# duanzhiihao/myDetection

Measured on AMD Instinct MI355X. Metric: images/sec at batch 32, 640x640, YOLOv3-80 (backbone -> FPN -> head -> decode -> NMS), higher is better.
Workload: dtype f32; 1 GPU; yolov3_80 (Darknet-53 + YOLOv3 FPN/head + decode + conf 0.005/top-512/NMS 0.45), batch 32/GPU, 640x640, random-init calibrated weights, hipGraph replay (1 batch lane per GPU); global_batch=32, image_size=640, parallelism=dp1, batch_lanes=1, batch_lanes_rule=model.batch_lanes_hint, passes=153, exchange=none

## Files before the change

include/mydet.h:

```cpp
#ifndef MYDET_H
#define MYDET_H

#include <stdint.h>

#ifdef __cplusplus
extern "C" {
#endif

#define MYDET_ABI_VERSION 2

#define MYDET_E_BADARG   (-1)
#define MYDET_E_UNSUPP   (-2)

#define MYDET_ACT_NONE   0
#define MYDET_ACT_LEAKY  1
#define MYDET_ACT_SWISH  2

int mydet_abi_version(void);

int mydet_conv2d_igemm_f32(const float *x, int64_t ldx, const float *w,
                           const float *scale, const float *shift,
                           const float *residual, int64_t ldr, const float *a_gate,
                           void *workspace, int64_t workspace_bytes,
                           float *y, int64_t ldy,
                           int B, int H, int W, int Cin, int Cout,
                           int KH, int KW, int stride, int pad_t, int pad_l,
                           int Ho, int Wo, int act, void *stream);

int64_t mydet_wino_weights_floats(int Cout, int Cin);
int mydet_wino_weights_f32(const float *w_ohwi, int Cout, int Cin, float *u, void *stream);
int mydet_conv2d_wino_f32(const float *x, int64_t ldx, const float *u, const float *scale, const float *shift,
                          const float *residual, int64_t ldr, void *workspace, int64_t workspace_bytes, float *y,
                          int64_t ldy, int B, int H, int W, int Cin, int Cout, int act, void *stream);

int mydet_conv2d_stem_f32(const float *x, int64_t sxb, int64_t sxc, int64_t sxh, int64_t sxw,
                          const float *w ,
                          const float *scale, const float *shift,
                          float *y, int64_t ldy,
                          int B, int H, int W, int Cout, int stride, int pad_t, int pad_l,
                          int Ho, int Wo, int act, void *stream);

#define MYDET_SE_EPOCH_WORDS 1024
typedef struct {
    const float *w1, *b1, *w2t, *b2;
    float *gate, *hpart;
    int Cse;
    int64_t hpart_bytes;
} mydet_se_tail;
int mydet_dwconv_slices(int Ho, int Wo, int C, int K, int stride);
int mydet_dwconv_se_groups(int Ho, int Wo, int C, int K, int stride);
int mydet_dwconv_f32(const float *x, int64_t ldx, const float *w, const float *scale, const float *shift,
                     float *y, int64_t ldy, int B, int H, int W, int C, int K, int stride, int pad_t, int pad_l,
                     int Ho, int Wo, int act, float *se_partial, int S, const mydet_se_tail *se, void *stream);

int mydet_channel_sums_f32(const float *x, int64_t ldx, int B, int H, int W, int C, float *partial, int S,
                           void *stream);

int mydet_se_gate_f32(float *partial, int S, int B, int HW, int C, const float *w1, const float *b1, int Cse,
                      const float *w2t, const float *b2, float *gate, void *stream);

int mydet_maxpool3s2_f32(const float *x, int64_t ldx, float *y, int64_t ldy, int B, int H, int W, int C,
                         int Ho, int Wo, void *stream);

int mydet_bifpn_fuse_f32(int n, const float *in0, int64_t ld0, int mode0, const float *in1, int64_t ld1, int mode1,
                         const float *in2, int64_t ld2, int mode2, const float *weights, float *y, int64_t ldy,
                         int B, int H, int W, int C, void *stream);

int mydet_upsample_concat_f32(const float *a, int64_t lda, int Ha, int Wa, int C1,
                              const float *b, int64_t ldb, int C2,
                              float *y, int64_t ldy, int B, int Ho, int Wo, void *stream);

int mydet_conv1x1_upcat_f32(const float *x_lo, int64_t ld_lo, int C_lo, const float *x_hi, int64_t ld_hi, int C_hi,
                            const float *w, const float *scale, const float *shift, void *workspace,
                            int64_t workspace_bytes, float *y, int64_t ldy, int B, int H, int W, int Cout, int act,
                            void *stream);

int64_t mydet_split_bf16_elems(int Cout, int K);
int mydet_split_bf16_f32(const float *w, int Cout, int K, uint16_t *planes, void *stream);
int mydet_conv2d_igemm_b3_f32(const float *x, int64_t ldx, const uint16_t *w_planes, const float *scale, const float *shift,
                              const float *residual, int64_t ldr, const float *a_gate, void *workspace, int64_t workspace_bytes, float *y,
                              int64_t ldy, int B, int H, int W, int Cin, int Cout, int KH, int KW, int stride, int pad_t,
                              int pad_l, int Ho, int Wo, int act, void *stream);
int mydet_conv3x3_p3_f32(const float *x, int64_t ldx, const uint16_t *w_planes, const float *scale, const float *shift,
                         const float *residual, int64_t ldr, float *y, int64_t ldy, int B, int H, int W, int Cin, int Cout,
                         int stride, int act, void *stream);
int mydet_conv_b3_reload_tuning(void);

int mydet_conv_igemm_occupancy(int cfg, int *assumed);

int mydet_space_to_depth_f32(const float *x, int64_t sb, int64_t sc, int64_t sh, int64_t sw, float *y, int64_t ldy,
                             int B, int C, int H, int W, void *stream);

int mydet_spp_concat_f32(const float *x, int64_t ldx, float *y, int64_t ldy, int B, int H, int W, int C, int k0, int k1,
                         int k2, void *stream);

#define MYDET_DECODE_YOLO   0
#define MYDET_DECODE_RETINA 1
#define MYDET_DECODE_FCOS   2
#define MYDET_DECODE_RAPID  3
typedef struct mydet_decode_level {
    const float *box; int64_t ldbox;
    const float *cls; int64_t ldcls;
    const float *anchors_wh;
    int H, W;
    float stride;
    int64_t n_off;
} mydet_decode_level;
int mydet_decode_levels_f32(int mode, int nlevels, const mydet_decode_level *levels, int box_astride, int box_c0,
                            int cls_astride, int cls_c0, int conf_c0, int A, int C, int B, int img_h, int img_w,
                            float *bbox, int64_t *class_idx, float *score, int64_t N, void *stream);
int mydet_decode_uv5_levels_f32(int nlevels, const mydet_decode_level *levels, int box_astride, int box_c0,
                                int cls_astride, int cls_c0, int conf_c0, int A, int C, int B, int img_h, int img_w,
                                float *bbox, int64_t *class_idx, float *score, int64_t N, void *stream);
int mydet_decode_f32(int mode,
                     const float *box, int64_t ldbox, int box_astride, int box_c0,
                     const float *cls, int64_t ldcls, int cls_astride, int cls_c0, int conf_c0,
                     const float *anchors_wh, int A, int C,
                     int B, int H, int W, float stride, int img_h, int img_w,
                     float *bbox, int64_t *class_idx, float *score, int64_t N, int64_t n_off,
                     void *stream);

int mydet_postprocess_f32(const float *bbox, const int64_t *class_idx, const float *score,
                          int B, int64_t N, float conf_thres, double nms_thres, int topk,
                          int32_t *count, float *out_bbox, int64_t *out_class, float *out_score,
                          int32_t *out_index, void *scratch, void *stream);

#define MYDET_COUNT_BAD_CLASS (-1)
#define MYDET_REC_TOPK   512
#define MYDET_REC_COUNT  0
#define MYDET_REC_BBOX   4
#define MYDET_REC_SCORE  (MYDET_REC_BBOX + 4 * MYDET_REC_TOPK)
#define MYDET_REC_CLASS  (MYDET_REC_SCORE + MYDET_REC_TOPK)
#define MYDET_REC_INDEX  (MYDET_REC_CLASS + 2 * MYDET_REC_TOPK)
#define MYDET_REC_WORDS  (MYDET_REC_INDEX + MYDET_REC_TOPK)
int mydet_postprocess_records_f32(const float *bbox, const int64_t *class_idx, const float *score,
                                  int B, int64_t N, float conf_thres, double nms_thres,
                                  int32_t *records, void *scratch, void *stream);

#define MYDET_REC_ANGLE     MYDET_REC_WORDS
#define MYDET_REC_ROT_WORDS (MYDET_REC_WORDS + MYDET_REC_TOPK)
int mydet_postprocess_rot_f32(const float *bbox, const int64_t *class_idx, const float *score,
                              int B, int64_t N, float conf_thres, double nms_thres, int topk,
                              int32_t *count, float *out_bbox, int64_t *out_class, float *out_score,
                              int32_t *out_index, void *scratch, void *stream);
int mydet_postprocess_records_rot_f32(const float *bbox, const int64_t *class_idx, const float *score,
                                      int B, int64_t N, float conf_thres, double nms_thres,
                                      int32_t *records, void *scratch, void *stream);

int64_t mydet_wino4_weights_floats(int Cout, int Cin);
int mydet_wino4_weights_f32(const float *w, int Cout, int Cin, float *u, void *stream);
int64_t mydet_wino4_workspace_bytes(int B, int H, int W, int Cin, int Cout);
int mydet_wino4_reload_tuning(void);
int mydet_conv2d_wino4_f32(const float *x, int64_t ldx, const float *u, const float *scale, const float *shift,
                           const float *residual, int64_t ldr, float *ws, int64_t ws_bytes, float *y, int64_t ldy,
                           int B, int H, int W, int Cin, int Cout, int act, void *stream);
int mydet_wino4_tail_plan(int B, int H, int W, int Cin, int Cout, int slots, int32_t *out);

int mydet_resize_bilinear_u8(const unsigned char *src, int H, int W, int64_t src_row_bytes, unsigned char *dst, int oh,
                             int ow, int64_t dst_row_bytes, const int32_t *bounds_x, const int32_t *kx, int ksx,
                             const int32_t *bounds_y, const int32_t *ky, int ksy, void *stream);

int mydet_bboxes_to_original_batched_f32(float *bbox, int64_t bbox_stride, const int32_t *count, int64_t count_stride,
                                         int B, int K, const float *pad_info, void *stream);
int mydet_detections_to_json_f64(const float *bbox, int64_t bbox_stride, const float *score, int64_t score_stride,
                                 const int64_t *cls, int64_t cls_stride, const int32_t *count, int64_t count_stride,
                                 int B, int K, const int64_t *cat_table, int n_cat, double *out, int64_t *out_cat,
                                 void *stream);

// ... 68 lines not shown
```

mydetection_amd/_lib.py:

```python
import ctypes
import os

_HERE = os.path.dirname(os.path.abspath(__file__))
LIB_PATH = os.environ.get('MYDET_LIB_PATH') or os.path.join(_HERE, 'lib', 'libmydet_hip.so')

c_int, c_i64, c_f32, c_f64, c_ptr = ctypes.c_int, ctypes.c_int64, ctypes.c_float, ctypes.c_double, ctypes.c_void_p

SIGNATURES = {
    'mydet_abi_version': [],
    'mydet_conv2d_igemm_f32': [c_ptr, c_i64, c_ptr, c_ptr, c_ptr, c_ptr, c_i64, c_ptr, c_ptr, c_i64, c_ptr, c_i64]
    + [c_int] * 13 + [c_ptr],
    'mydet_wino_weights_floats': [c_int, c_int],
    'mydet_wino_weights_f32': [c_ptr, c_int, c_int, c_ptr, c_ptr],
    'mydet_conv2d_wino_f32': [c_ptr, c_i64, c_ptr, c_ptr, c_ptr, c_ptr, c_i64, c_ptr, c_i64, c_ptr, c_i64] + [c_int] * 6
    + [c_ptr],
    'mydet_wino4_weights_floats': [c_int, c_int],
    'mydet_wino4_weights_f32': [c_ptr, c_int, c_int, c_ptr, c_ptr],
    'mydet_wino4_workspace_bytes': [c_int, c_int, c_int, c_int, c_int],
    'mydet_wino4_reload_tuning': [],
    'mydet_conv_b3_reload_tuning': [],
    'mydet_conv_igemm_occupancy': [c_int, c_ptr],
    'mydet_split_bf16_elems': [c_int, c_int],
    'mydet_split_bf16_f32': [c_ptr, c_int, c_int, c_ptr, c_ptr],
    'mydet_conv2d_igemm_b3_f32': [c_ptr, c_i64, c_ptr, c_ptr, c_ptr, c_ptr, c_i64, c_ptr, c_ptr, c_i64, c_ptr, c_i64] + [c_int] * 13 + [c_ptr],
    'mydet_conv3x3_p3_f32': [c_ptr, c_i64, c_ptr, c_ptr, c_ptr, c_ptr, c_i64, c_ptr, c_i64] + [c_int] * 7 + [c_ptr],
    'mydet_wino4_tail_plan': [c_int, c_int, c_int, c_int, c_int, c_int, c_ptr],
    'mydet_conv2d_wino4_f32': [c_ptr, c_i64, c_ptr, c_ptr, c_ptr, c_ptr, c_i64, c_ptr, c_i64, c_ptr, c_i64] + [c_int] * 6 + [c_ptr],
    'mydet_dwconv_slices': [c_int, c_int, c_int, c_int, c_int],
    'mydet_dwconv_se_groups': [c_int, c_int, c_int, c_int, c_int],
    'mydet_dwconv_f32': [c_ptr, c_i64, c_ptr, c_ptr, c_ptr, c_ptr, c_i64] + [c_int] * 11 + [c_ptr, c_int, c_ptr, c_ptr],
    'mydet_channel_sums_f32': [c_ptr, c_i64, c_int, c_int, c_int, c_int, c_ptr, c_int, c_ptr],
    'mydet_se_gate_f32': [c_ptr, c_int, c_int, c_int, c_int, c_ptr, c_ptr, c_int, c_ptr, c_ptr, c_ptr, c_ptr],
    'mydet_maxpool3s2_f32': [c_ptr, c_i64, c_ptr, c_i64] + [c_int] * 6 + [c_ptr],
    'mydet_bifpn_fuse_f32': [c_int, c_ptr, c_i64, c_int, c_ptr, c_i64, c_int, c_ptr, c_i64, c_int, c_ptr, c_ptr, c_i64,
                             c_int, c_int, c_int, c_int, c_ptr],
    'mydet_conv2d_stem_f32': [c_ptr, c_i64, c_i64, c_i64, c_i64, c_ptr, c_ptr, c_ptr, c_ptr, c_i64] + [c_int] * 10 + [c_ptr],
    'mydet_upsample_concat_f32': [c_ptr, c_i64, c_int, c_int, c_int, c_ptr, c_i64, c_int, c_ptr, c_i64, c_int, c_int,
                                  c_int, c_ptr],
    'mydet_conv1x1_upcat_f32': [c_ptr, c_i64, c_int, c_ptr, c_i64, c_int, c_ptr, c_ptr, c_ptr, c_ptr, c_i64, c_ptr, c_i64]
    + [c_int] * 5 + [c_ptr],
    'mydet_space_to_depth_f32': [c_ptr, c_i64, c_i64, c_i64, c_i64, c_ptr, c_i64, c_int, c_int, c_int, c_int, c_ptr],
    'mydet_spp_concat_f32': [c_ptr, c_i64, c_ptr, c_i64] + [c_int] * 7 + [c_ptr],
    'mydet_decode_levels_f32': [c_int, c_int, c_ptr, c_int, c_int, c_int, c_int, c_int, c_int, c_int, c_int, c_int, c_int,
                                c_ptr, c_ptr, c_ptr, c_i64, c_ptr],
    'mydet_decode_uv5_levels_f32': [c_int, c_ptr, c_int, c_int, c_int, c_int, c_int, c_int, c_int, c_int, c_int, c_int,
                                    c_ptr, c_ptr, c_ptr, c_i64, c_ptr],
    'mydet_decode_f32': [c_int, c_ptr, c_i64, c_int, c_int, c_ptr, c_i64, c_int, c_int, c_int, c_ptr, c_int, c_int,
                         c_int, c_int, c_int, c_f32, c_int, c_int, c_ptr, c_ptr, c_ptr, c_i64, c_i64, c_ptr],
    'mydet_postprocess_f32': [c_ptr, c_ptr, c_ptr, c_int, c_i64, c_f32, c_f64, c_int, c_ptr, c_ptr, c_ptr, c_ptr,
                              c_ptr, c_ptr, c_ptr],
    'mydet_postprocess_records_f32': [c_ptr, c_ptr, c_ptr, c_int, c_i64, c_f32, c_f64, c_ptr, c_ptr, c_ptr],
    'mydet_postprocess_rot_f32': [c_ptr, c_ptr, c_ptr, c_int, c_i64, c_f32, c_f64, c_int, c_ptr, c_ptr, c_ptr, c_ptr,
                                  c_ptr, c_ptr, c_ptr],
    'mydet_postprocess_records_rot_f32': [c_ptr, c_ptr, c_ptr, c_int, c_i64, c_f32, c_f64, c_ptr, c_ptr, c_ptr],
    'mydet_mbconv_tiles': [c_int, c_int, c_int],
    'mydet_mbconv_expand_dw_f32': [c_ptr, c_i64, c_ptr, c_ptr, c_ptr, c_ptr, c_ptr, c_i64] + [c_int] * 11 + [c_ptr, c_int, c_ptr, c_ptr],
    'mydet_sepconv_nodes_f32': [c_int, c_ptr, c_int, c_int, c_ptr],
    'mydet_stem_dw_f32': [c_ptr, c_i64, c_i64, c_i64, c_i64, c_ptr, c_ptr, c_ptr, c_ptr, c_ptr, c_i64, c_int, c_int, c_int, c_int,
                          c_int, c_int, c_int, c_int, c_ptr, c_int, c_ptr, c_ptr],
    'mydet_lr_tb_levels_f32': [c_int, c_ptr, c_int, c_int, c_ptr],
    'mydet_sepconv_decode_retina_f32': [c_int, c_ptr, c_int, c_int, c_int, c_int, c_int, c_int, c_ptr, c_ptr, c_ptr, c_i64, c_ptr],
    'mydet_bboxes_iou_f32': [c_ptr, c_int, c_ptr, c_int, c_int, c_ptr, c_ptr],
    'mydet_bboxes_to_original_batched_f32': [c_ptr, c_i64, c_ptr, c_i64, c_int, c_int, c_ptr, c_ptr],
    'mydet_detections_to_json_f64': [c_ptr, c_i64, c_ptr, c_i64, c_ptr, c_i64, c_ptr, c_i64, c_int, c_int, c_ptr, c_int, c_ptr, c_ptr, c_ptr],
    'mydet_resize_bilinear_u8': [c_ptr, c_int, c_int, c_i64, c_ptr, c_int, c_int, c_i64, c_ptr, c_ptr, c_int, c_ptr, c_ptr, c_int, c_ptr],
    'mydet_preprocess_u8_f32': [c_ptr, c_int, c_int, c_int, c_ptr, c_int, c_int, c_int, c_ptr, c_ptr, c_ptr],
    'mydet_cxcywh_to_x1y1x2y2_f32': [c_ptr, c_ptr, c_i64, c_int, c_ptr],
    'mydet_bboxes_to_original_f32': [c_ptr, c_i64, c_f32, c_f32, c_f32, c_f32, c_f32, c_f32, c_ptr],
}



RETURNS_I64 = {'mydet_wino_weights_floats', 'mydet_wino4_weights_floats', 'mydet_wino4_workspace_bytes', 'mydet_split_bf16_elems'}

REC_TOPK = 512
REC_COUNT, REC_BBOX = 0, 4
REC_SCORE = REC_BBOX + 4 * REC_TOPK
REC_CLASS = REC_SCORE + REC_TOPK
REC_INDEX = REC_CLASS + 2 * REC_TOPK
REC_WORDS = REC_INDEX + REC_TOPK
REC_ANGLE = REC_WORDS
REC_ROT_WORDS = REC_WORDS + REC_TOPK


class DecodeLevel(ctypes.Structure):
    _fields_ = [('box', c_ptr), ('ldbox', c_i64), ('cls', c_ptr), ('ldcls', c_i64), ('anchors_wh', c_ptr),
                ('H', c_int), ('W', c_int), ('stride', c_f32), ('n_off', c_i64)]


class SeTail(ctypes.Structure):
    _fields_ = [('w1', c_ptr), ('b1', c_ptr), ('w2t', c_ptr), ('b2', c_ptr), ('gate', c_ptr), ('hpart', c_ptr), ('Cse', c_int),
                ('hpart_bytes', c_i64)]


SE_EPOCH_WORDS = 1024
ABI_VERSION = 2


class SepconvNode(ctypes.Structure):
    _fields_ = [('inp', c_ptr * 3), ('ld', c_i64 * 3), ('mode', c_int * 3), ('n_in', c_int), ('fuse_weights', c_ptr),
                ('w_dw', c_ptr), ('w_pw_packed', c_ptr), ('scale', c_ptr), ('shift', c_ptr), ('y', c_ptr), ('ldy', c_i64),
                ('H', c_int), ('W', c_int), ('Cout', c_int), ('act', c_int)]


class SepconvDecodeNode(ctypes.Structure):
    _fields_ = [('node', SepconvNode), ('kind', c_int), ('stride', c_f32), ('anchors_wh', c_ptr), ('n_off', c_i64)]


# ... 47 lines not shown
```

mydetection_amd/models/backbones.py:

```python
import torch.nn as nn

from .. import ops
from .modules import ConvBn, ConvBnLeaky, DarkBlock


class Darknet53(nn.Module):
    def __init__(self, global_cfg):
        super().__init__()
        self.netlist = nn.ModuleList()
        in_ch = global_cfg.get('model.backbone.input_channels', 3)
        self.netlist.append(ConvBnLeaky(in_ch, 32, k=3, s=1))
        width = 32
        for n_blocks in (1, 2, 8, 8, 4):
            self.netlist.append(ConvBnLeaky(width, width * 2, k=3, s=2))
            width *= 2
            for _ in range(n_blocks):
                self.netlist.append(DarkBlock(in_out=width, hidden=width // 2))
        assert len(self.netlist) == 29

    def forward(self, x):
        feats = []
        for i, layer in enumerate(self.netlist):
            x = layer(x)
            if i in (14, 23, 28):
                feats.append(x)
        return feats


class UltralyticsBackbone(nn.Module):
    def __init__(self, global_cfg):
        super().__init__()
        import math
        from ..external.ultralytics.common import Focus, Bottleneck, BottleneckCSP, Conv, SPP
        depm = global_cfg['model.ultralytics.depth_muliple']
        chm = global_cfg['model.ultralytics.channel_muliple']
        ch = [int(math.ceil(c * chm / 8) * 8) for c in (64, 128, 256, 512, 1024)]

        def reps(n):
            return max(round(n * depm), 1)
        self.feature_chs = ch[2:]
        self.feature_strides = [8, 16, 32]
        self.netlist = nn.ModuleList()
        if global_cfg['model.ultralytics.first'] == 'Focus':
            assert global_cfg.get('general.input.frame_concatenation', 1) == 1
            self.netlist.append(Focus(3, ch[0], k=3))
        else:
            raise NotImplementedError()
        self.netlist.append(Conv(ch[0], ch[1], k=3, s=2))
        self.netlist.append(nn.Sequential(*[Bottleneck(ch[1], ch[1]) for _ in range(reps(3))]))
        self.netlist.append(Conv(ch[1], ch[2], k=3, s=2))
        self.netlist.append(BottleneckCSP(ch[2], ch[2], n=reps(9)))
        self.netlist.append(Conv(ch[2], ch[3], k=3, s=2))
        self.netlist.append(BottleneckCSP(ch[3], ch[3], n=reps(9)))
        self.netlist.append(Conv(ch[3], ch[4], k=3, s=2))
        self.netlist.append(SPP(ch[4], ch[4], k=[5, 9, 13]))
        self.netlist.append(BottleneckCSP(ch[4], ch[4], n=reps(6)))

    def forward(self, x):
        assert x.dim() == 4 and x.shape[2] % 32 == 0 and x.shape[3] % 32 == 0
        features = []
        for module in self.netlist:
            y = module(x)
            if y.shape[2:4] != x.shape[2:4]:
                assert y.shape[2] == x.shape[2] // 2
                features.append(x)
            x = y
        features.append(x)
        assert len(features) == 6
        return features[3:]


class _PoolAfter(ConvBn):
    def __init__(self, in_ch, out_ch, k, padding):
        super().__init__(in_ch, out_ch, k, padding)
        self.add_module('2', nn.MaxPool2d(3, stride=2, padding=1))

    def forward(self, x):
        return ops.maxpool3s2(ConvBn.forward(self, x))


class _MaxPool(nn.Module):
    def forward(self, x):
        return ops.maxpool3s2(x)


class EfNetBackbone(nn.Module):
    valid_names = {'efficientnet-b0', 'efficientnet-b1', 'efficientnet-b2', 'efficientnet-b3', 'efficientnet-b4',
                   'efficientnet-b5', 'efficientnet-b6'}

    def __init__(self, cfg: dict):
        super().__init__()
        model_name = cfg['model.backbone.name']
        assert model_name in self.valid_names, 'Unknown efficientnet model name'
        from ..external.efficientnet.model import EfficientNet
        efn = EfficientNet.from_name(model_name)
        self.model = efn
        efnet_chs = [efn._blocks_args[i].output_filters for i in [2, 4, 6]]
        if cfg['model.backbone.num_levels'] == 3:
            self.feature_chs = efnet_chs
            self.feature_strides = (8, 16, 32)
            self.C6C7 = False
        elif cfg['model.backbone.num_levels'] == 5:
            out_ch = cfg['model.backbone.C6C7_out_channels']
            downsample_layer = cfg.get('model.efficientnet.C6C7_downsample', 'maxpool')
            if downsample_layer == 'maxpool':
# ... 35 lines not shown
```

mydetection_amd/models/modules.py:

```python
import torch
import torch.nn as nn

from .. import ops


def _versions(*tensors):
    return tuple((t.data_ptr(), t._version) for t in tensors)


def prepare_conv(owner, slot, conv, bn, depthwise=False):
    tensors = [conv.weight] + ([bn.weight, bn.bias, bn.running_mean, bn.running_var] if bn is not None else [])
    if conv.bias is not None:
        tensors.append(conv.bias)
    key = _versions(*tensors)
    cache = owner.__dict__.setdefault('_prep_cache', {})
    hit = cache.get(slot)
    if hit is None or hit[0] != key:
        with torch.no_grad():
            w = conv.weight.detach().float()
            if depthwise:
                w = w.permute(2, 3, 0, 1).reshape(w.shape[2], w.shape[3], w.shape[0]).contiguous()
            else:
                w = w.permute(0, 2, 3, 1).contiguous()
            if bn is not None:
                inv = (bn.running_var.float() + bn.eps).sqrt().reciprocal()
                scale = (bn.weight.float() * inv).contiguous()
                shift = (bn.bias.float() - bn.running_mean.float() * scale).contiguous()
                if conv.bias is not None:
                    shift = (shift + conv.bias.float() * scale).contiguous()
            else:
                scale = None
                shift = conv.bias.detach().float().contiguous() if conv.bias is not None else None
        hit = (key, (w, scale, shift))
        cache[slot] = hit
    return hit[1]


def prepare_wino(owner, slot, w_ohwi):
    cache = owner.__dict__.setdefault('_prep_cache', {})
    hit = cache.get(slot)
    if hit is None or hit[0] is not w_ohwi:
        u = ops.wino_weights(w_ohwi) if ops.WINOGRAD else None
        u4 = ops.wino4_weights(w_ohwi) if ops.WINOGRAD and ops.WINOGRAD4 and w_ohwi.shape[3] >= ops.WINO4_MIN_CIN else None
        hit = (w_ohwi, (u, u4))
        cache[slot] = hit
    return hit[1]


def prepare_b3(owner, slot, w_ohwi):
    if not ops.SPLIT_BF16 or (w_ohwi.shape[3] % 16 and not (w_ohwi.shape[1] == 1 and w_ohwi.shape[2] == 1 and w_ohwi.shape[3] % 4 == 0)):
        return None
    cache = owner.__dict__.setdefault('_prep_cache', {})
    hit = cache.get(slot)
    if hit is None or hit[0] is not w_ohwi:
        hit = (w_ohwi, ops.split_bf16(w_ohwi))
        cache[slot] = hit
    return hit[1]


class FusedConvMixin:

    def _prepared(self, conv, bn):
        return prepare_conv(self, 'main', conv, bn)


class ConvBnLeaky(nn.Module, FusedConvMixin):
    def __init__(self, c1, c2, k=1, s=1):
        super().__init__()
        self.k, self.s = k, s
        self.conv = nn.Conv2d(c1, c2, k, s, padding=(k - 1) // 2, bias=False)
        self.bn = nn.BatchNorm2d(c2, eps=1e-5, momentum=0.01)

    def forward(self, x, residual=None, upcat_lo=None):
        if self.training:
            raise NotImplementedError('mydetection_amd implements the inference path only; call model.eval()')
        w, scale, shift = self._prepared(self.conv, self.bn)
        p = (self.k - 1) // 2
        if upcat_lo is not None:
            assert residual is None
            if self.k == 1 and self.s == 1:
                y = ops.conv1x1_upcat(upcat_lo, x, w, scale, shift, ops.ACT_LEAKY)
                if y is not None:
                    return y
            x = ops.upsample_concat(upcat_lo, tuple(x.shape[2:4]), x)
        if w.shape[3] == 3 and self.k == 3 and w.shape[0] == 32 and residual is None:
            return ops.conv2d_stem(x, w, scale, shift, self.s, (p, p, p, p), ops.ACT_LEAKY)
        u, u4 = prepare_wino(self, 'wino', w) if self.k == 3 and self.s == 1 else (None, None)
        b3 = prepare_b3(self, 'b3', w) if (u is None and u4 is None) or (self.k == 3 and w.shape[3] <= ops.P3_S1_MAX_CIN) else None
        return ops.conv2d(x, w, scale, shift, self.k, self.s, (p, p, p, p), ops.ACT_LEAKY, residual=residual, wino=u, wino4=u4, b3=b3)


class DarkBlock(nn.Module):
    def __init__(self, in_out, hidden):
        super().__init__()
        self.cbl_0 = ConvBnLeaky(in_out, hidden, k=1, s=1)
        self.cbl_1 = ConvBnLeaky(hidden, in_out, k=3, s=1)

    def forward(self, x):
        return self.cbl_1(self.cbl_0(x), residual=x)


class Swish(nn.Module):
    def forward(self, x):
        raise NotImplementedError('Swish is fused into the producing conv kernel on the inference path')


class SeparableConv2d(nn.Module):
    def __init__(self, in_ch, out_ch, kernel_size, stride, padding):
        super().__init__()
        self.k, self.s, self.p = kernel_size, stride, padding
        self.depthwise = nn.Conv2d(in_ch, in_ch, kernel_size, stride, padding=padding, groups=in_ch, bias=False)
        self.pointwise = nn.Conv2d(in_ch, out_ch, 1, 1, padding=0)

    def fusable(self):
        return (ops.FUSED_NODES and self.k == 3 and self.s == 1 and self.p == 1
                and self.depthwise.in_channels in ops.SEPCONV_CHANNELS and self.pointwise.out_channels % 4 == 0)

    def node(self, inputs, modes=None, fuse_weights=None, bn=None, act=ops.ACT_NONE, out=None):
        if self.training:
            raise NotImplementedError('mydetection_amd implements the inference path only; call model.eval()')
        wd, _, _ = prepare_conv(self, 'dw', self.depthwise, None, depthwise=True)
        wp, scale, shift = prepare_conv(self, ('pw', id(bn)), self.pointwise, bn)
        cache = self.__dict__.setdefault('_prep_cache', {})
        hit = cache.get(('pwk', id(bn)))
        if hit is None or hit[0] is not wp:
            hit = (wp, ops.pack_pointwise(wp))
            cache[('pwk', id(bn))] = hit
        return dict(inputs=list(inputs), modes=modes, fuse_weights=fuse_weights, w_dw=wd, w_pw=hit[1], scale=scale,
                    shift=shift, cout=self.pointwise.out_channels, act=act, out=out)

    def node_per_anchor(self, inputs, A, n_cls):
        nd = self.node(inputs)
        wp, _, shift = prepare_conv(self, ('pw', id(None)), self.pointwise, None)
        cache = self.__dict__.setdefault('_prep_cache', {})
        hit = cache.get(('pwk_anchor', A, n_cls))
        if hit is None or hit[0] is not wp:
            hit = (wp, ops.pack_pointwise_per_anchor(wp, shift, A, n_cls))
            cache[('pwk_anchor', A, n_cls)] = hit
        nd['w_pw'], nd['shift'] = hit[1]
        return nd

    def forward(self, x, bn=None, act=ops.ACT_NONE):
        if self.training:
            raise NotImplementedError('mydetection_amd implements the inference path only; call model.eval()')
        if self.fusable():
            return ops.sepconv_nodes([self.node([x], bn=bn, act=act)])[0]
        wd, _, _ = prepare_conv(self, 'dw', self.depthwise, None, depthwise=True)
        x = ops.dwconv(x, wd, None, None, self.k, self.s, (self.p,) * 4, ops.ACT_NONE)
        wp, scale, shift = prepare_conv(self, ('pw', id(bn)), self.pointwise, bn)
        return ops.conv2d(x, wp, scale, shift, 1, 1, (0, 0, 0, 0), act)


class ConvBn(nn.Sequential):
    def __init__(self, in_ch, out_ch, k=1, padding=0, eps=0.001):
        super().__init__(nn.Conv2d(in_ch, out_ch, k, stride=1, padding=padding),
                         nn.BatchNorm2d(out_ch, eps=eps, momentum=0.01))
        self.k, self.p = k, padding

    def forward(self, x):
        w, scale, shift = prepare_conv(self, 'main', self[0], self[1])
        u, u4 = prepare_wino(self, 'wino', w) if self.k == 3 and self.p == 1 else (None, None)
        return ops.conv2d(x, w, scale, shift, self.k, 1, (self.p,) * 4, ops.ACT_NONE, wino=u, wino4=u4)


class SpconvBn(nn.Sequential):
    def __init__(self, ch, swish):
        mods = [SeparableConv2d(ch, ch, 3, 1, padding=1), nn.BatchNorm2d(ch, eps=0.001, momentum=0.01)]
        if swish:
            mods.append(Swish())
        super().__init__(*mods)
        self.act = ops.ACT_SWISH if swish else ops.ACT_NONE

    def fusable(self):
        return self[0].fusable()
# ... 7 lines not shown
```

mydetection_amd/ops.py:

```python
import ctypes
import os
import threading

import numpy as np
import torch

from . import _lib

ACT_NONE, ACT_LEAKY, ACT_SWISH = 0, 1, 2
DECODE_YOLO, DECODE_RETINA, DECODE_FCOS, DECODE_RAPID = 0, 1, 2, 3
TOPK = 512


def _stream():
    return ctypes.c_void_p(torch.cuda.current_stream().cuda_stream)


class KernelTimer:

    def __init__(self, chain=False):
        self.spans = {}
        self.bytes = {}
        self.fused = {}
        self.chain = chain
# ... 305 lines not shown
            TIMER.stop(name, t0, 2.0 * B * Ho * Wo * Cout * 9 * Cin,
                       4.0 * (B * H * W * Cin + B * Ho * Wo * Cout * (2 if residual is not None else 1) + 9 * Cin * Cout))
        _lib.check(code, 'mydet_conv2d_wino_f32')
        return out
    ws = conv_workspace(x.device)
    if (b3 is not None and b3_takes(B * Ho * Wo, Cin, Cout, k, b3_min_rows, min_cout=B3_GATED_MIN_COUT if gate is not None else 128)
            and (gate is None or (k == 1 and act == ACT_NONE))):
        t0 = TIMER.start() if TIMER else None
        code = _lib.lib().mydet_conv2d_igemm_b3_f32(
            _ptr(x), ldx, _ptr(b3), _ptr(scale), _ptr(shift), _ptr(residual), ldr, _ptr(gate), _ptr(ws), ws.numel() * 4, _ptr(out), ldy,
            B, H, W, Cin, Cout, k, k, stride, pad[0], pad[1], Ho, Wo, act, _stream())
        if code != -2:
            if t0:
                name = f'conv_igemm_b3 {Cin}->{Cout} k{k}s{stride} {H}x{W}' if TIMER_DETAIL else 'conv_igemm_b3'
                b_in, b_out = 4.0 * B * H * W * Cin, 4.0 * B * Ho * Wo * Cout
                b_rest = 4.0 * (k * k * Cin * Cout) + (b_out if residual is not None else 0.0)
                TIMER.stop(name, t0, 2.0 * B * Ho * Wo * Cout * k * k * Cin, b_in + b_out + b_rest)
            _lib.check(code, 'mydet_conv2d_igemm_b3_f32')
            return out
    t0 = TIMER.start() if TIMER else None
    code = _lib.lib().mydet_conv2d_igemm_f32(
        _ptr(x), ldx, _ptr(w_ohwi), _ptr(scale), _ptr(shift), _ptr(residual), ldr, _ptr(gate),
        _ptr(ws), ws.numel() * 4 if ws is not None else 0, _ptr(out), ldy,
        B, H, W, Cin, Cout, k, k, stride, pad[0], pad[1], Ho, Wo, act, _stream())
    if t0:
        name = f'conv_igemm {Cin}->{Cout} k{k}s{stride} {H}x{W}' if TIMER_DETAIL else 'conv_igemm'
        b_in, b_out = 4.0 * B * H * W * Cin, 4.0 * B * Ho * Wo * Cout
        b_rest = 4.0 * (k * k * Cin * Cout) + (b_out if residual is not None else 0.0)
        TIMER.stop(name, t0, 2.0 * B * Ho * Wo * Cout * k * k * Cin, b_in + b_out + b_rest,
                   (0.0 if interior == 'in' else b_in) + (0.0 if interior == 'out' else b_out) + b_rest)
    _lib.check(code, 'mydet_conv2d_igemm_f32')
    return out


def conv3x3_p3(x, b3, scale, shift, stride, act, residual=None, out=None, out_ld=None, cout=None):
    require_gpu(x, 'conv3x3_p3')
    x, ldx = to_nhwc(x)
    B, Cin, H, W = x.shape
    Cout = int(cout if cout is not None else (shift if shift is not None else scale).shape[0])
    if Cin % 16 or stride not in (1, 2) or act not in (ACT_NONE, ACT_LEAKY) or b3 is None:
        return None
    Ho, Wo = (H - 1) // stride + 1, (W - 1) // stride + 1
    if out is None:
        out, ldy = empty_nhwc(B, Cout, Ho, Wo, x.device, out_ld)
    else:
        ldy = nhwc_ld(out)
        assert ldy is not None and out.shape == (B, Cout, Ho, Wo)
    ldr = 0
    if residual is not None:
        residual, ldr = to_nhwc(residual)
        assert residual.shape == out.shape
    t0 = TIMER.start() if TIMER else None
    code = _lib.lib().mydet_conv3x3_p3_f32(_ptr(x), ldx, _ptr(b3), _ptr(scale), _ptr(shift), _ptr(residual), ldr, _ptr(out), ldy,
                                           B, H, W, Cin, Cout, stride, act, _stream())
    if code == -2:
        return None
    if t0:
        name = f'conv_p3 {Cin}->{Cout} k3s{stride} {H}x{W}' if TIMER_DETAIL else 'conv_p3'
        b_in, b_out = 4.0 * B * H * W * Cin, 4.0 * B * Ho * Wo * Cout
        TIMER.stop(name, t0, 2.0 * B * Ho * Wo * Cout * 9 * Cin, b_in + b_out + 4.0 * 9 * Cin * Cout + (b_out if residual is not None else 0.0))
    _lib.check(code, 'mydet_conv3x3_p3_f32')
    return out


def conv2d_stem(x, w_ohwi, scale, shift, stride, pad, act):
    require_gpu(x, 'conv2d_stem')
    assert x.dtype == torch.float32 and x.shape[1] == 3
    B, _, H, W = x.shape
    Cout = w_ohwi.shape[0]
    Ho = conv_out_size(H, 3, stride, pad[0], pad[2])
    Wo = conv_out_size(W, 3, stride, pad[1], pad[3])
    out, ldy = empty_nhwc(B, Cout, Ho, Wo, x.device)
    sb, sc, sh, sw = x.stride()
    t0 = TIMER.start() if TIMER else None
    code = _lib.lib().mydet_conv2d_stem_f32(_ptr(x), sb, sc, sh, sw, _ptr(w_ohwi), _ptr(scale), _ptr(shift),
                                            _ptr(out), ldy, B, H, W, Cout, stride, pad[0], pad[1], Ho, Wo, act,
                                            _stream())
    if t0:
        TIMER.stop('conv_stem', t0, *[4.0 * B * (3 * H * W + Cout * Ho * Wo)] * 2)
    _lib.check(code, 'mydet_conv2d_stem_f32')
    return out


def se_slices(n_pixels):
    return max(1, min(128, n_pixels // 16))


def dwconv(x, w_kkc, scale, shift, k, stride, pad, act, squeeze=False, interior=False, se=None):
    require_gpu(x, 'dwconv')
    x, ldx = to_nhwc(x)
    B, C, H, W = x.shape
    Ho = conv_out_size(H, k, stride, pad[0], pad[2])
    Wo = conv_out_size(W, k, stride, pad[1], pad[3])
    out, ldy = empty_nhwc(B, C, Ho, Wo, x.device)
    partial, S = None, 0
    if squeeze or se is not None:
        S = _lib.lib().mydet_dwconv_slices(Ho, Wo, C, k, stride)
    if squeeze:
        partial = torch.empty((B, S + 1, C), dtype=torch.float32, device=x.device)
    tail, gate, keep = _se_tail(se, B, C, _lib.lib().mydet_dwconv_se_groups(Ho, Wo, C, k, stride) if se is not None else 0, x.device)
    t0 = TIMER.start() if TIMER else None
    code = _lib.lib().mydet_dwconv_f32(_ptr(x), ldx, _ptr(w_kkc), _ptr(scale), _ptr(shift), _ptr(out), ldy, B, H, W, C,
                                       k, stride, pad[0], pad[1], Ho, Wo, act, _ptr(partial), S,
                                       ctypes.byref(tail) if tail is not None else None, _stream())
    if t0:
        TIMER.stop(f'dwconv {C} k{k}s{stride} {H}x{W}' if TIMER_DETAIL else 'dwconv', t0, *[4.0 * B * C * (H * W + Ho * Wo)] * 2,
                   fused=0.0 if interior is True else (4.0 * B * C * H * W if interior == 'out' else None))
    _lib.check(code, 'mydet_dwconv_f32')
    if se is not None:
        return out, gate
    return (out, partial) if squeeze else out


MBCONV_FUSED_SHAPES = {(3, 2, 16), (3, 1, 24), (5, 2, 24)}
FUSED_MBCONV = os.environ.get('MYDET_FUSED_MBCONV', '1') != '0'


def fold_scale(w, scale):
    if w.dim() == 3:
        return (w * scale.view(1, 1, -1)).contiguous()
    return (w * scale.view(-1, *([1] * (w.dim() - 1)))).contiguous()


def mbconv_expand_dw(x, w_expand, shift0, w_dw, shift1, k, stride, pad, se=None):
    require_gpu(x, 'mbconv_expand_dw')
    x, ldx = to_nhwc(x)
    B, Cin, H, W = x.shape
    Cexp = w_expand.shape[0]
    Ho = conv_out_size(H, k, stride, pad[0], pad[2])
    Wo = conv_out_size(W, k, stride, pad[1], pad[3])
    out, ldy = empty_nhwc(B, Cexp, Ho, Wo, x.device)
    S = _lib.lib().mydet_mbconv_tiles(Ho, Wo, stride)
    partial = torch.empty((B, S + 1, Cexp), dtype=torch.float32, device=x.device) if se is None else None
    tail, gate, keep = _se_tail(se, B, Cexp, S, x.device)
    t0 = TIMER.start() if TIMER else None
    code = _lib.lib().mydet_mbconv_expand_dw_f32(_ptr(x), ldx, _ptr(w_expand), _ptr(shift0), _ptr(w_dw),
                                                 _ptr(shift1), _ptr(out), ldy, B, H, W, Cin, Cexp, k, stride,
                                                 pad[0], pad[1], Ho, Wo, _ptr(partial), S,
                                                 ctypes.byref(tail) if tail is not None else None, _stream())
    if t0:
        nb = 4.0 * B * (H * W * (Cin + Cexp) + Cexp * (H * W + Ho * Wo))
        TIMER.stop(f'mbconv_expand_dw {Cin}->{Cexp} k{k}s{stride} {H}x{W}' if TIMER_DETAIL else 'mbconv_expand_dw', t0,
                   2.0 * B * H * W * Cin * Cexp, nb, fused=4.0 * B * H * W * Cin)
    _lib.check(code, 'mydet_mbconv_expand_dw_f32')
    return (out, gate) if se is not None else (out, partial)


FUSED_STEM_DW = os.environ.get('MYDET_FUSED_STEM', '1') != '0'


def stem_dw(x, w_stem, shift0, w_dw, shift1, pad, se=None):
    require_gpu(x, 'stem_dw')
    assert x.dtype == torch.float32 and x.shape[1] == 3
    B, _, H, W = x.shape
    C = w_stem.shape[0]
    Hs = conv_out_size(H, 3, 2, pad[0], pad[2])
    Ws = conv_out_size(W, 3, 2, pad[1], pad[3])
    out, ldy = empty_nhwc(B, C, Hs, Ws, x.device)
    S = _lib.lib().mydet_mbconv_tiles(Hs, Ws, 1)
    partial = torch.empty((B, S + 1, C), dtype=torch.float32, device=x.device) if se is None else None
    tail, gate, keep = _se_tail(se, B, C, S, x.device)
    sb, sc, sh, sw = x.stride()
    t0 = TIMER.start() if TIMER else None
    code = _lib.lib().mydet_stem_dw_f32(_ptr(x), sb, sc, sh, sw, _ptr(w_stem), _ptr(shift0), _ptr(w_dw), _ptr(shift1), _ptr(out),
                                        ldy, B, H, W, C, pad[0], pad[1], Hs, Ws, _ptr(partial), S,
                                        ctypes.byref(tail) if tail is not None else None, _stream())
# ... 578 lines not shown
```

Baseline: 1608 images/sec.

## Fuse Darknet stem 3x3 conv and stride-2 3x3 conv into one kernel

Adds a kernel that computes the first 3x3 stride-1 conv (3->32 channels) on an LDS-staged input patch using split-bf16 MFMA. It keeps the 32-channel activation in LDS as three bf16 planes and feeds it straight into the following 3x3 stride-2 conv, also on MFMA. This removes the write and re-read of the full-resolution 32-channel feature map in global memory and saves one launch. The cost is a large LDS footprint with low occupancy, recomputation of halo pixels per output tile, and three-plane bf16 emulation of f32 precision.

```diff
diff --git a/include/mydet.h b/include/mydet.h
--- a/include/mydet.h
+++ b/include/mydet.h
@@ -84,6 +84,11 @@
 int mydet_conv3x3_p3_f32(const float *x, int64_t ldx, const uint16_t *w_planes, const float *scale, const float *shift,
                          const float *residual, int64_t ldr, float *y, int64_t ldy, int B, int H, int W, int Cin, int Cout,
                          int stride, int act, void *stream);
+int mydet_conv_stem_p3_f32(const float *x, int64_t sxb, int64_t sxc, int64_t sxh, int64_t sxw, const uint16_t *w0_planes,
+                           const float *scale0, const float *shift0, int act0, const uint16_t *w1_planes, const float *scale1,
+                           const float *shift1, int act1, float *y, int64_t ldy, int B, int H, int W, int C0, int Cout,
+                           int stride0, int pad_t, int pad_l, int Hs, int Ws, int stride1, void *stream);
+int mydet_conv_stem_p3_lds_bytes(void);
 int mydet_conv_b3_reload_tuning(void);
 
 int mydet_conv_igemm_occupancy(int cfg, int *assumed);
diff --git a/mydetection_amd/_lib.py b/mydetection_amd/_lib.py
--- a/mydetection_amd/_lib.py
+++ b/mydetection_amd/_lib.py
@@ -24,6 +24,9 @@
     'mydet_split_bf16_f32': [c_ptr, c_int, c_int, c_ptr, c_ptr],
     'mydet_conv2d_igemm_b3_f32': [c_ptr, c_i64, c_ptr, c_ptr, c_ptr, c_ptr, c_i64, c_ptr, c_ptr, c_i64, c_ptr, c_i64] + [c_int] * 13 + [c_ptr],
     'mydet_conv3x3_p3_f32': [c_ptr, c_i64, c_ptr, c_ptr, c_ptr, c_ptr, c_i64, c_ptr, c_i64] + [c_int] * 7 + [c_ptr],
+    'mydet_conv_stem_p3_f32': [c_ptr, c_i64, c_i64, c_i64, c_i64, c_ptr, c_ptr, c_ptr, c_int, c_ptr, c_ptr, c_ptr, c_int, c_ptr, c_i64]
+    + [c_int] * 11 + [c_ptr],
+    'mydet_conv_stem_p3_lds_bytes': [],
     'mydet_wino4_tail_plan': [c_int, c_int, c_int, c_int, c_int, c_int, c_ptr],
     'mydet_conv2d_wino4_f32': [c_ptr, c_i64, c_ptr, c_ptr, c_ptr, c_ptr, c_i64, c_ptr, c_i64, c_ptr, c_i64] + [c_int] * 6 + [c_ptr],
     'mydet_dwconv_slices': [c_int, c_int, c_int, c_int, c_int],
diff --git a/mydetection_amd/csrc/conv_stem_p3.hip b/mydetection_amd/csrc/conv_stem_p3.hip
--- /dev/null
+++ b/mydetection_amd/csrc/conv_stem_p3.hip
@@ -0,0 +1,317 @@
+#include "common.h"
+
+namespace {
+
+constexpr unsigned OOB = 0xFFFFFFFFu;
+constexpr int SP_COUT_PAD = 256;
+
+constexpr int SP_PH = 17, SP_PW = 33, SP_ROWLEN = 36, SP_PJ0 = 17, SP_ROWB = 32;
+constexpr int SP_NPIX = SP_PH * SP_PW;
+constexpr int SP_NBLK = (SP_NPIX + 31) / 32;
+constexpr int SP_BPW = (SP_NBLK + 3) / 4;
+constexpr int SP_PLANE = SP_PH * SP_ROWLEN * SP_ROWB;
+constexpr int SP_SLAB = 3 * SP_PLANE;
+constexpr int SP_IH = SP_PH + 2, SP_IW = SP_PW + 2, SP_ILD = 36;
+constexpr int SP_ICH = SP_IH * SP_ILD;
+constexpr int SP_LDS = SP_SLAB + 3 * SP_ICH * 4;
+
+struct StemP3Args {
+    const float *x, *scale0, *shift0, *scale, *shift;
+    const unsigned short *w0, *wsplit;
+    float *y;
+    int64_t sxb, sxc, sxh, sxw, ldy;
+    int B, H, W, pad_t, pad_l, Hs, Ws, act0, Cout, Ho, Wo;
+    int tx_n, ntn, nblk, tiles_img;
+};
+
+typedef __bf16 bf16x8 __attribute__((ext_vector_type(8)));
+typedef __bf16 bf16x4 __attribute__((ext_vector_type(4)));
+
+__device__ __forceinline__ __amdgpu_buffer_rsrc_t sp_rsrc(const void *base, int64_t bytes) {
+    const uint64_t a = (uint64_t)base;
+    const unsigned lo = __builtin_amdgcn_readfirstlane((unsigned)a);
+    const unsigned hi = __builtin_amdgcn_readfirstlane((unsigned)(a >> 32));
+    const int64_t capped = bytes > 0x7FFFFFF0ll ? 0x7FFFFFF0ll : bytes;
+    const int n = __builtin_amdgcn_readfirstlane((int)capped);
+    return __builtin_amdgcn_make_buffer_rsrc((void *)(((uint64_t)hi << 32) | lo), 0, n, 0x00020000);
+}
+
+__device__ __forceinline__ void sp_split1(const float v, __bf16 &p0, __bf16 &p1, __bf16 &p2) {
+    const __bf16 h0 = (__bf16)v;
+    const float r1 = v - (float)h0;
+    const __bf16 h1 = (__bf16)r1;
+    const float r2 = r1 - (float)h1;
+    p0 = h0; p1 = h1; p2 = (__bf16)r2;
+}
+
+__device__ __forceinline__ int sp_pos(int py, int px) { return py * SP_ROWLEN + (px & 1) * SP_PJ0 + (px >> 1); }
+__device__ __forceinline__ int sp_sigma(int px) { return ((px >> 1) >> 3) & 1; }
+
+__device__ __forceinline__ void sp_store_quad(char *patch, int pos, int sig, int half, int fh, const float (&v)[4]) {
+    bf16x4 q0, q1, q2;
+#pragma unroll
+    for (int e = 0; e < 4; ++e) {
+        __bf16 h0, h1, h2;
+        sp_split1(v[e], h0, h1, h2);
+        q0[e] = h0; q1[e] = h1; q2[e] = h2;
+    }
+    char *d = patch + pos * SP_ROWB + ((half ^ sig) * 16) + fh * 8;
+    *reinterpret_cast<bf16x4 *>(d) = q0;
+    *reinterpret_cast<bf16x4 *>(d + SP_PLANE) = q1;
+    *reinterpret_cast<bf16x4 *>(d + 2 * SP_PLANE) = q2;
+}
+
+template <int ACT>
+__global__ __launch_bounds__(256, 2) void conv_stem_p3_kernel(const StemP3Args p) {
+    extern __shared__ __attribute__((aligned(16))) char smem_sp[];
+    constexpr int TWL = 4, TW = 16, RPB = 2, TM = 2, WN = 2;
+    char *patch = smem_sp;
+    float *img = reinterpret_cast<float *>(smem_sp + SP_SLAB);
+
+    const int id = mydet_xcd_remap(blockIdx.x, p.nblk);
+    const int nt = id % p.ntn, t = id / p.ntn;
+    const int b = t / p.tiles_img, rt = t - b * p.tiles_img;
+    const int ty = rt / p.tx_n, tx = rt - ty * p.tx_n;
+    const int oy0 = ty * 8, ox0 = tx * 16, n0 = nt * 64;
+    const int sy0 = 2 * oy0 - 1, sx0 = 2 * ox0 - 1;
+    const int tid = threadIdx.x;
+    const int wave = tid >> 6, lane = tid & 63;
+    const int wm = wave / WN, wn = wave % WN;
+    const int fr = lane & 31, fh = lane >> 5;
+
+    {
+        const float *xb = p.x + (int64_t)b * p.sxb;
+        const int iy0 = sy0 - p.pad_t, ix0 = sx0 - p.pad_l;
+        constexpr int NE = 3 * SP_IH * SP_IW, NI = (NE + 255) / 256;
+        float v[NI];
+#pragma unroll
+        for (int i = 0; i < NI; ++i) {
+            const int e = tid + 256 * i;
+            const int c = e / (SP_IH * SP_IW), rem = e - c * (SP_IH * SP_IW);
+            const int r = rem / SP_IW, q = rem - r * SP_IW;
+            const int iy = iy0 + r, ix = ix0 + q;
+            const bool ok = e < NE && (unsigned)iy < (unsigned)p.H && (unsigned)ix < (unsigned)p.W;
+            v[i] = ok ? xb[c * p.sxc + (int64_t)iy * p.sxh + (int64_t)ix * p.sxw] : 0.0f;
+        }
+#pragma unroll
+        for (int i = 0; i < NI; ++i) {
+            const int e = tid + 256 * i;
+            const int c = e / (SP_IH * SP_IW), rem = e - c * (SP_IH * SP_IW);
+            const int r = rem / SP_IW, q = rem - r * SP_IW;
+            if (e < NE) img[c * SP_ICH + r * SP_ILD + q] = v[i];
+        }
+    }
+
+    const unsigned unit = (unsigned)((2 * fr + (fh ^ ((fr >> 2) & 1))) * 16);
+    const int CoutP = (p.Cout + SP_COUT_PAD - 1) / SP_COUT_PAD * SP_COUT_PAD;
+    const __amdgpu_buffer_rsrc_t wr = sp_rsrc(p.wsplit, (int64_t)9 * 2 * 3 * CoutP * 32);
+    const unsigned boff = (unsigned)((n0 + wn * 32) * 32) + unit;
+    const unsigned plane_bytes = (unsigned)CoutP * 32u, slab_bytes = 3u * plane_bytes;
+
+    float keep[SP_BPW][8];
+    {
+        const __amdgpu_buffer_rsrc_t w0r = sp_rsrc(p.w0, (int64_t)2 * 3 * SP_COUT_PAD * 32);
+        bf16x8 wf[2][3];
+#pragma unroll
+        for (int ks = 0; ks < 2; ++ks)
+#pragma unroll
+            for (int pl = 0; pl < 3; ++pl)
+                wf[ks][pl] = __builtin_bit_cast(bf16x8, __builtin_amdgcn_raw_buffer_load_b128(w0r, unit, (ks * 3 + pl) * SP_COUT_PAD * 32, 0));
+        float sc0[16], sh0[16];
+#pragma unroll
+        for (int r = 0; r < 16; ++r) {
+            const int ch = (r & 3) + 8 * (r >> 2) + 4 * fh;
+            sc0[r] = p.scale0 ? p.scale0[ch] : 1.0f;
+            sh0[r] = p.shift0 ? p.shift0[ch] : 0.0f;
+        }
+        int koff[16];
+#pragma unroll
+        for (int j = 0; j < 16; ++j) {
+            const int ka = 16 * (j >> 3) + (j & 7), kb = ka + 8;
+            const int ta = ka / 3, tb = kb / 3;
+            const int oa = (ka - 3 * ta) * SP_ICH + (ta / 3) * SP_ILD + ta % 3;
+            const int ob = kb < 27 ? (kb - 3 * tb) * SP_ICH + (tb / 3) * SP_ILD + tb % 3 : 0;
+            koff[j] = fh ? ob : oa;
+        }
+        __syncthreads();
+
+#pragma unroll
+        for (int bi = 0; bi < SP_BPW; ++bi) {
+            const int blk = wave + 4 * bi;
+            if (blk < SP_NBLK) {
+                const int m_raw = blk * 32 + fr;
+                const bool mok = m_raw < SP_NPIX;
+                const int m = mok ? m_raw : SP_NPIX - 1;
+                const int py = m / SP_PW, px = m - py * SP_PW;
+                const float *ib = img + py * SP_ILD + px;
+                bf16x8 pa[2][3];
+#pragma unroll
+                for (int j = 0; j < 16; ++j) {
+                    float v = ib[koff[j]];
+                    if (j >= 11 && fh) v = 0.0f;
+                    __bf16 h0, h1, h2;
+                    sp_split1(v, h0, h1, h2);
+                    pa[j >> 3][0][j & 7] = h0; pa[j >> 3][1][j & 7] = h1; pa[j >> 3][2][j & 7] = h2;
+                }
+                f32x16 acc;
+#pragma unroll
+                for (int r = 0; r < 16; ++r) acc[r] = 0.f;
+                constexpr int PA[6] = {2, 1, 0, 1, 0, 0}, PB[6] = {0, 1, 2, 0, 1, 0};
+#pragma unroll
+                for (int ks = 0; ks < 2; ++ks)
+#pragma unroll
+                    for (int tt = 0; tt < 6; ++tt)
+                        acc = __builtin_amdgcn_mfma_f32_32x32x16_bf16(wf[ks][PB[tt]], pa[ks][PA[tt]], acc, 0, 0, 0);
+                const int sy = sy0 + py, sx = sx0 + px;
+                const bool inside = (unsigned)sy < (unsigned)p.Hs && (unsigned)sx < (unsigned)p.Ws;
+                const int pos = sp_pos(py, px), sig = sp_sigma(px);
+#pragma unroll
+                for (int g = 0; g < 4; ++g) {
+                    float o[4];
+#pragma unroll
+                    for (int e = 0; e < 4; ++e) {
+                        const int r = 4 * g + e;
+                        o[e] = inside ? mydet_act(acc[r] * sc0[r] + sh0[r], p.act0) : 0.0f;
+                    }
+                    if (g < 2) {
+                        if (mok) sp_store_quad(patch, pos, sig, g & 1, fh, o);
+                    } else {
+#pragma unroll
+                        for (int e = 0; e < 4; ++e) keep[bi][(g - 2) * 4 + e] = o[e];
+                    }
+                }
+            }
+        }
+    }
+
+    const int oxl = fr & (TW - 1);
+    int apos[TM], apy[TM];
+#pragma unroll
+    for (int i = 0; i < TM; ++i) {
+        const int oyl = wm * (TM * RPB) + i * RPB + (fr >> TWL);
+        apy[i] = 2 * oyl;
+        apos[i] = apy[i] * SP_ROWLEN + oxl;
+    }
+    f32x16 acc[TM];
+#pragma unroll
+    for (int i = 0; i < TM; ++i)
+#pragma unroll
+        for (int r = 0; r < 16; ++r) acc[i][r] = 0.f;
+    const int nch = n0 + wn * 32 + fr;
+    const float pscl = p.scale ? p.scale[nch < p.Cout ? nch : 0] : 1.0f;
+    const float psft = p.shift ? p.shift[nch < p.Cout ? nch : 0] : 0.0f;
+
+    bf16x8 breg[3][3];
+    auto load_b = [&](int cs, int tap, bf16x8 (&brg)[3]) {
+        const unsigned kt = (unsigned)(tap * 2 + cs);
+#pragma unroll
+        for (int pl = 0; pl < 3; ++pl)
+            brg[pl] = __builtin_bit_cast(bf16x8, __builtin_amdgcn_raw_buffer_load_b128(wr, cs < 2 ? boff : OOB,
+                                                     __builtin_amdgcn_readfirstlane(kt * slab_bytes + (unsigned)pl * plane_bytes), 0));
+    };
+    auto compute = [&](int tap, const bf16x8 (&bf)[3]) {
+        const int kh = tap / 3, kw = tap - kh * 3;
+        bf16x8 af[TM][3];
+#pragma unroll
+        for (int i = 0; i < TM; ++i) {
+            const int pos = apos[i] + kh * SP_ROWLEN + (kw & 1) * SP_PJ0 + (kw >> 1);
+            const int sig = ((oxl + (kw >> 1)) >> 3) & 1;
+            const char *a = patch + pos * SP_ROWB + ((fh ^ sig) * 16);
+#pragma unroll
+            for (int pl = 0; pl < 3; ++pl) af[i][pl] = *reinterpret_cast<const bf16x8 *>(a + pl * SP_PLANE);
+        }
+        constexpr int PA[6] = {2, 1, 0, 1, 0, 0}, PB[6] = {0, 1, 2, 0, 1, 0};
+#pragma unroll
+        for (int tt = 0; tt < 6; ++tt)
+#pragma unroll
+            for (int i = 0; i < TM; ++i)
+                acc[i] = __builtin_amdgcn_mfma_f32_32x32x16_bf16(af[i][PA[tt]], bf[PB[tt]], acc[i], 0, 0, 0);
+    };
+
+    load_b(0, 0, breg[0]);
+    load_b(0, 1, breg[1]);
+    load_b(0, 2, breg[2]);
+#pragma unroll
+    for (int cs = 0; cs < 2; ++cs) {
+        if (cs == 1) {
+            mydet_lds_barrier();
+#pragma unroll
+            for (int bi = 0; bi < SP_BPW; ++bi) {
+                const int m = (wave + 4 * bi) * 32 + fr;
+                if (m < SP_NPIX) {
+                    const int py = m / SP_PW, px = m - py * SP_PW;
+                    const int pos = sp_pos(py, px), sig = sp_sigma(px);
+#pragma unroll
+                    for (int g = 0; g < 2; ++g) {
+                        const float o[4] = {keep[bi][4 * g], keep[bi][4 * g + 1], keep[bi][4 * g + 2], keep[bi][4 * g + 3]};
+                        sp_store_quad(patch, pos, sig, g, fh, o);
+                    }
+                }
+            }
+        }
+        mydet_lds_barrier();
+#pragma unroll
+        for (int tap = 0; tap < 9; ++tap) {
+            compute(tap, breg[tap % 3]);
+            const int t3 = tap + 3;
+            load_b(cs + t3 / 9, t3 % 9, breg[tap % 3]);
+        }
+    }
+
+    const int64_t opix = (int64_t)p.Ho * p.Wo;
+    const __amdgpu_buffer_rsrc_t yr = sp_rsrc(p.y + b * opix * p.ldy, opix * p.ldy * 4);
+    const unsigned ldy4 = (unsigned)p.ldy * 4u;
+    const bool nok = nch < p.Cout;
+#pragma unroll
+    for (int i = 0; i < TM; ++i) {
+        const int oyb = oy0 + wm * (TM * RPB) + i * RPB;
+#pragma unroll
+        for (int r = 0; r < 16; ++r) {
+            const int dr = (r & 3) + 8 * (r >> 2) + 4 * fh;
+            const int oy = oyb + (dr >> TWL), ox = ox0 + (dr & (TW - 1));
+            const bool ok = nok && oy < p.Ho && ox < p.Wo;
+            const unsigned off = ok ? (unsigned)(oy * p.Wo + ox) * ldy4 + (unsigned)nch * 4u : OOB;
+            float v = acc[i][r] * pscl + psft;
+            if (ACT == MYDET_ACT_LEAKY) v = v > 0.0f ? v : v * 0.1f;
+            __builtin_amdgcn_raw_buffer_store_b32(__builtin_bit_cast(unsigned, v), yr, off, 0, 0);
+        }
+    }
+}
+
+template <int ACT>
+int sp_launch(const StemP3Args &p, hipStream_t st) {
+    static unsigned long long mask = 0;
+    auto kern = &conv_stem_p3_kernel<ACT>;
+    const int rc = mydet_lds_opt_in(mask, kern, SP_LDS);
+    if (rc != 0) return rc;
+    hipLaunchKernelGGL(kern, dim3(p.nblk), dim3(256), SP_LDS, st, p);
+    return mydet_launch_status();
+}
+
+}
+
+extern "C" int mydet_conv_stem_p3_lds_bytes(void) { return SP_LDS; }
+
+extern "C" int mydet_conv_stem_p3_f32(const float *x, int64_t sxb, int64_t sxc, int64_t sxh, int64_t sxw, const uint16_t *w0_planes,
+                                      const float *scale0, const float *shift0, int act0, const uint16_t *w1_planes, const float *scale1,
+                                      const float *shift1, int act1, float *y, int64_t ldy, int B, int H, int W, int C0, int Cout,
+                                      int stride0, int pad_t, int pad_l, int Hs, int Ws, int stride1, void *stream) {
+    if (!x || !w0_planes || !w1_planes || !y || B <= 0 || H <= 0 || W <= 0 || Hs <= 0 || Ws <= 0 || Cout <= 0) return MYDET_E_BADARG;
+    if (C0 != 32 || (Cout & 63) || stride0 != 1 || stride1 != 2) return MYDET_E_UNSUPP;
+    if ((act0 != MYDET_ACT_NONE && act0 != MYDET_ACT_LEAKY) || (act1 != MYDET_ACT_NONE && act1 != MYDET_ACT_LEAKY)) return MYDET_E_UNSUPP;
+    if ((ldy & 3) || ldy < Cout || ((uintptr_t)y & 15)) return MYDET_E_BADARG;
+    if (((uintptr_t)w0_planes & 15) || ((uintptr_t)w1_planes & 15) || ((uintptr_t)x & 3)) return MYDET_E_BADARG;
+    StemP3Args p;
+    p.x = x; p.scale0 = scale0; p.shift0 = shift0; p.scale = scale1; p.shift = shift1; p.w0 = w0_planes; p.wsplit = w1_planes; p.y = y;
+    p.sxb = sxb; p.sxc = sxc; p.sxh = sxh; p.sxw = sxw; p.ldy = ldy;
+    p.B = B; p.H = H; p.W = W; p.pad_t = pad_t; p.pad_l = pad_l; p.Hs = Hs; p.Ws = Ws; p.act0 = act0; p.Cout = Cout;
+    p.Ho = (Hs - 1) / 2 + 1; p.Wo = (Ws - 1) / 2 + 1;
+    if ((int64_t)p.Ho * p.Wo * ldy * 4 > 0x7FFFFFF0ll) return MYDET_E_UNSUPP;
+    p.tx_n = (p.Wo + 15) / 16; p.ntn = Cout / 64;
+    p.tiles_img = p.tx_n * ((p.Ho + 7) / 8);
+    const int64_t nblk = (int64_t)B * p.tiles_img * p.ntn;
+    if (nblk > 0x7FFFFFFF || nblk <= 0) return MYDET_E_UNSUPP;
+    p.nblk = (int)nblk;
+    hipStream_t st = (hipStream_t)stream;
+    return act1 == MYDET_ACT_LEAKY ? sp_launch<MYDET_ACT_LEAKY>(p, st) : sp_launch<MYDET_ACT_NONE>(p, st);
+}
diff --git a/mydetection_amd/models/backbones.py b/mydetection_amd/models/backbones.py
--- a/mydetection_amd/models/backbones.py
+++ b/mydetection_amd/models/backbones.py
@@ -1,7 +1,7 @@
 import torch.nn as nn
 
 from .. import ops
-from .modules import ConvBn, ConvBnLeaky, DarkBlock
+from .modules import ConvBn, ConvBnLeaky, DarkBlock, stem_p3
 
 
 class Darknet53(nn.Module):
@@ -20,7 +20,11 @@
 
     def forward(self, x):
         feats = []
+        y = stem_p3(self.netlist[0], self.netlist[1], x)
         for i, layer in enumerate(self.netlist):
+            if y is not None and i < 2:
+                x = y
+                continue
             x = layer(x)
             if i in (14, 23, 28):
                 feats.append(x)
diff --git a/mydetection_amd/models/modules.py b/mydetection_amd/models/modules.py
--- a/mydetection_amd/models/modules.py
+++ b/mydetection_amd/models/modules.py
@@ -90,6 +90,24 @@
         return ops.conv2d(x, w, scale, shift, self.k, self.s, (p, p, p, p), ops.ACT_LEAKY, residual=residual, wino=u, wino4=u4, b3=b3)
 
 
+def stem_p3(cbl_0, cbl_1, x):
+    if (cbl_0.training or cbl_1.training or (cbl_0.k, cbl_0.s, cbl_1.k, cbl_1.s) != (3, 1, 3, 2) or x.dim() != 4 or x.shape[1] != 3
+            or cbl_0.conv.out_channels != 32 or cbl_1.conv.in_channels != 32 or x.dtype != torch.float32 or not x.is_cuda
+            or cbl_0._forward_hooks or cbl_0._forward_pre_hooks or cbl_1._forward_hooks or cbl_1._forward_pre_hooks):
+        return None
+    B, _, H, W = x.shape
+    if not (ops.SPLIT_BF16 and ops.stem_p3_takes(B, H, W, cbl_1.conv.out_channels, (1, 1, 1, 1))):
+        return None
+    w0, scale0, shift0 = cbl_0._prepared(cbl_0.conv, cbl_0.bn)
+    w1, scale1, shift1 = cbl_1._prepared(cbl_1.conv, cbl_1.bn)
+    cache = cbl_0.__dict__.setdefault('_prep_cache', {})
+    hit = cache.get('stem_p3')
+    if hit is None or hit[0] is not w0:
+        hit = (w0, ops.stem_p3_weights(w0))
+        cache['stem_p3'] = hit
+    return ops.conv_stem_p3(x, hit[1], scale0, shift0, (1, 1, 1, 1), prepare_b3(cbl_1, 'b3', w1), scale1, shift1)
+
+
 class DarkBlock(nn.Module):
     def __init__(self, in_out, hidden):
         super().__init__()
diff --git a/mydetection_amd/ops.py b/mydetection_amd/ops.py
--- a/mydetection_amd/ops.py
+++ b/mydetection_amd/ops.py
@@ -411,6 +411,55 @@
     return out
 
 
+STEM_P3 = os.environ.get('MYDET_STEM_P3', '1') != '0'
+
+
+def stem_p3_plan(B, Hs, Ws, Cout):
+    Ho, Wo = (Hs - 1) // 2 + 1, (Ws - 1) // 2 + 1
+    return B * -(-Ho // 8) * -(-Wo // 16) * (Cout // 64), 3 * 17 * 36 * 32 + 3 * 19 * 36 * 4
+
+
+def stem_p3_takes(B, H, W, Cout, pad0):
+    Hs, Ws = conv_out_size(H, 3, 1, pad0[0], pad0[2]), conv_out_size(W, 3, 1, pad0[1], pad0[3])
+    Ho, Wo = (Hs - 1) // 2 + 1, (Ws - 1) // 2 + 1
+    if not STEM_P3 or Cout % 64 or not p3_takes(B, Ho, Wo, 32, Cout, 3, 2, (1, 1, 1, 1)):
+        return False
+    return not (P3_STRIP and Wo % 16 in (4, 8))
+
+
+def stem_p3_weights(w_ohwi):
+    w = torch.zeros((w_ohwi.shape[0], 1, 1, 32), dtype=torch.float32, device=w_ohwi.device)
+    w[:, 0, 0, :27] = w_ohwi.reshape(w_ohwi.shape[0], 27).float()
+    return split_bf16(w)
+
+
+def conv_stem_p3(x, w0_planes, scale0, shift0, pad0, w1_planes, scale1, shift1, act0=ACT_LEAKY, act1=ACT_LEAKY, out=None, out_ld=None):
+    require_gpu(x, 'conv_stem_p3')
+    assert x.dtype == torch.float32 and x.shape[1] == 3
+    B, _, H, W = x.shape
+    Cout = int(shift1.shape[0])
+    Hs, Ws = conv_out_size(H, 3, 1, pad0[0], pad0[2]), conv_out_size(W, 3, 1, pad0[1], pad0[3])
+    Ho, Wo = (Hs - 1) // 2 + 1, (Ws - 1) // 2 + 1
+    if out is None:
+        out, ldy = empty_nhwc(B, Cout, Ho, Wo, x.device, out_ld)
+    else:
+        ldy = nhwc_ld(out)
+        assert ldy is not None and out.shape == (B, Cout, Ho, Wo)
+    sb, sc, sh, sw = x.stride()
+    t0 = TIMER.start() if TIMER else None
+    code = _lib.lib().mydet_conv_stem_p3_f32(_ptr(x), sb, sc, sh, sw, _ptr(w0_planes), _ptr(scale0), _ptr(shift0), act0, _ptr(w1_planes),
+                                             _ptr(scale1), _ptr(shift1), act1, _ptr(out), ldy, B, H, W, 32, Cout, 1, pad0[0], pad0[1],
+                                             Hs, Ws, 2, _stream())
+    if code == -2:
+        return None
+    if t0:
+        b_img, b_map, b_out = 4.0 * B * 3 * H * W, 4.0 * B * 32 * Hs * Ws, 4.0 * B * Cout * Ho * Wo
+        TIMER.stop('conv_stem_p3', t0, 2.0 * B * (Hs * Ws * 32 * 27 + Ho * Wo * Cout * 9 * 32), b_img + 2 * b_map + b_out + 4.0 * 9 * 32 * Cout,
+                   fused=b_img + b_out + 4.0 * 9 * 32 * Cout)
+    _lib.check(code, 'mydet_conv_stem_p3_f32')
+    return out
+
+
 def se_slices(n_pixels):
     return max(1, min(128, n_pixels // 16))
 
```

Result: faster. 1640 images/sec, median of 6 (+2.0%).
